# lacibeb/GA3C

Measured on NVIDIA B200. Metric: TPS: A3C training frames/s, NetworkVP 84x84x4 (PPS: predictions/s, in 'pps'), higher is better.
Workload: dtype bf16

## Files before the change

### experiments/microbench/umma_bench.cu

```cuda
#include <cstdio>
#include <cstdlib>
#include <cstdint>
#include <cuda_runtime.h>
#define CK(x) do { cudaError_t e = (x); if (e != cudaSuccess) { printf("CUDA error %s at %d\n", cudaGetErrorString(e), __LINE__); exit(1); } } while (0)

__device__ __forceinline__ uint32_t smem_u32(const void* p) { return (uint32_t)__cvta_generic_to_shared(p); }
__device__ __forceinline__ void mbar_init(uint32_t bar, uint32_t c) { asm volatile("mbarrier.init.shared::cta.b64 [%0], %1;\n" ::"r"(bar), "r"(c)); }
__device__ __forceinline__ void mbar_wait(uint32_t bar, uint32_t parity) {
  asm volatile("{\n.reg .pred p;\nW_%=:\nmbarrier.try_wait.parity.shared::cta.b64 p, [%0], %1;\n@p bra D_%=;\nbra W_%=;\nD_%=:\n}\n" ::"r"(bar), "r"(parity) : "memory");
}
__device__ __forceinline__ bool elect_one() {
  uint32_t pred;
  asm volatile("{\n.reg .pred p;\nelect.sync _|p, 0xffffffff;\nselp.u32 %0, 1, 0, p;\n}\n" : "=r"(pred));
  return pred != 0;
}
__device__ __forceinline__ void mma(uint32_t d, uint32_t a_lo, uint32_t a_hi, uint32_t b_lo, uint32_t b_hi, uint32_t idesc, uint32_t acc) {
  asm volatile("{\n.reg .pred p;\n.reg .b64 da, db;\nsetp.ne.b32 p, %6, 0;\nmov.b64 da, {%1, %2};\nmov.b64 db, {%3, %4};\n"
               "tcgen05.mma.cta_group::1.kind::f16 [%0], da, db, %5, p;\n}\n" ::"r"(d), "r"(a_lo), "r"(a_hi), "r"(b_lo), "r"(b_hi), "r"(idesc), "r"(acc) : "memory");
}
struct Cfg { int M, N, a_mn, b_mn, swz, nacc, a_lbo, a_sbo, b_lbo, b_sbo, a_step, b_step, nrot; };

__global__ void __launch_bounds__(128, 1) bench(Cfg c, int reps, long long* out) {
  extern __shared__ __align__(1024) uint8_t smem[];
  __shared__ __align__(8) unsigned long long bar_s;
  __shared__ uint32_t tslot;
  const uint32_t base = (smem_u32(smem) + 1023u) & ~1023u, bar = smem_u32(&bar_s);
  for (int i = threadIdx.x; i < 200 * 1024 / 16; i += blockDim.x) reinterpret_cast<uint4*>(smem)[i] = make_uint4(0, 0, 0, 0);
  if (threadIdx.x == 0) { mbar_init(bar, 1); asm volatile("fence.mbarrier_init.release.cluster;\n" ::: "memory"); }
  if (threadIdx.x < 32) {
    asm volatile("tcgen05.alloc.cta_group::1.sync.aligned.shared::cta.b32 [%0], 512;\n" ::"r"(smem_u32(&tslot)) : "memory");
    asm volatile("tcgen05.relinquish_alloc_permit.cta_group::1.sync.aligned;\n" ::: "memory");
  }
  asm volatile("fence.proxy.async.shared::cta;\n" ::: "memory");
  asm volatile("tcgen05.fence::before_thread_sync;\n" ::: "memory");
  __syncthreads();
  asm volatile("tcgen05.fence::after_thread_sync;\n" ::: "memory");
  const uint32_t tmem = tslot;
  const uint32_t idesc = (1u << 4) | (1u << 7) | (1u << 10) | ((uint32_t)c.a_mn << 15) | ((uint32_t)c.b_mn << 16) | ((uint32_t)(c.N >> 3) << 17) | ((uint32_t)(c.M >> 4) << 24);
  const uint32_t lay = c.swz ? (2u << 29) : 0u;
  const uint32_t a_base = base, b_base = base + 128 * 1024;
  const uint32_t a_lo0 = ((a_base & 0x3FFFFu) >> 4) | ((uint32_t)(c.a_lbo >> 4) << 16), a_hi = (uint32_t)(c.a_sbo >> 4) | (1u << 14) | lay;
  const uint32_t b_lo0 = ((b_base & 0x3FFFFu) >> 4) | ((uint32_t)(c.b_lbo >> 4) << 16), b_hi = (uint32_t)(c.b_sbo >> 4) | (1u << 14) | lay;
  long long t0 = 0, t1 = 0;
  if (threadIdx.x < 32) {
    for (int round = 0; round < 2; ++round) {
      t0 = clock64();
      if (elect_one()) {
        for (int i = 0; i < reps; ++i) {
          const int r = i % c.nrot;
          mma(tmem + (i % c.nacc) * c.N, a_lo0 + r * (c.a_step >> 4), a_hi, b_lo0 + r * (c.b_step >> 4), b_hi, idesc, 1u);
        }
        asm volatile("tcgen05.commit.cta_group::1.mbarrier::arrive::one.shared::cluster.b64 [%0];\n" ::"r"(bar) : "memory");
      }
      __syncwarp();
      mbar_wait(bar, round & 1);
      t1 = clock64();
    }
  }
  asm volatile("tcgen05.fence::before_thread_sync;\n" ::: "memory");
  __syncthreads();
  if (threadIdx.x == 0) out[blockIdx.x] = t1 - t0;
  if (threadIdx.x < 32) asm volatile("tcgen05.dealloc.cta_group::1.sync.aligned.b32 %0, 512;\n" ::"r"(tmem) : "memory");
}

int main() {
  long long* out; CK(cudaMalloc(&out, 8 * 148));
  CK(cudaFuncSetAttribute(bench, cudaFuncAttributeMaxDynamicSharedMemorySize, 201 * 1024 + 1024));
  const int reps = 2048;
  struct Named { const char* name; Cfg c; } tests[] = {
      {"wgrad11  M64  N16  A MN-ns  B MN-ns  4 acc", {64, 16, 1, 1, 0, 4, 128, 7872, 128, 7424, 256, 256, 16}},
      {"wgrad11  M64  N16  A MN-ns  B MN-ns  1 acc", {64, 16, 1, 1, 0, 1, 128, 7872, 128, 7424, 256, 256, 16}},
      {"wgrad12  M64  N32  A MN-ns  B MN-ns  4 acc", {64, 32, 1, 1, 0, 4, 128, 2560, 128, 2816, 256, 256, 8}},
      {"merged   M64  N64  A MN-ns  B MN-ns  1 acc", {64, 64, 1, 1, 0, 1, 128, 7872, 128, 7424, 256, 256, 16}},
      {"merged   M64  N128 A MN-ns  B MN-ns  1 acc", {64, 128, 1, 1, 0, 1, 128, 7872, 128, 4096, 256, 256, 8}},
      {"         M128 N16  A MN-ns  B MN-ns  4 acc", {128, 16, 1, 1, 0, 4, 128, 7872, 128, 7424, 256, 256, 16}},
      {"         M128 N64  A MN-ns  B MN-ns  1 acc", {128, 64, 1, 1, 0, 1, 128, 7872, 128, 7424, 256, 256, 16}},
      {"dgrad    M128 N64  A K-ns   B K-ns   2 acc", {128, 64, 0, 0, 0, 2, 2816, 128, 1024, 128, 16, 0, 8}},
      {"conv11f  M128 N32  A K-ns   B K-ns   4 acc", {128, 32, 0, 0, 0, 4, 8768, 128, 512, 128, 16, 0, 8}},
      {"         M128 N16  A K-ns   B K-ns   4 acc", {128, 16, 0, 0, 0, 4, 8768, 128, 512, 128, 16, 0, 8}},
      {"         M64  N16  A K-ns   B K-ns   4 acc", {64, 16, 0, 0, 0, 4, 8768, 128, 512, 128, 16, 0, 8}},
      {"conv12f  M128 N32  A K-sw128 B K-sw128 1 acc", {128, 32, 0, 0, 1, 1, 16, 1024, 16, 1024, 32, 32, 4}},
      {"         M128 N64  A K-sw128 B K-sw128 1 acc", {128, 64, 0, 0, 1, 1, 16, 1024, 16, 1024, 32, 32, 4}},
      {"         M128 N128 A K-sw128 B K-sw128 1 acc", {128, 128, 0, 0, 1, 1, 16, 1024, 16, 1024, 32, 32, 4}},
      {"         M128 N256 A K-sw128 B K-sw128 1 acc", {128, 256, 0, 0, 1, 1, 16, 1024, 16, 1024, 32, 32, 4}},
      {"         M64  N32  A K-sw128 B K-sw128 1 acc", {64, 32, 0, 0, 1, 1, 16, 1024, 16, 1024, 32, 32, 4}},
      {"         M64  N64  A MN-sw128 B MN-sw128 1 acc", {64, 64, 1, 1, 1, 1, 8192, 1024, 8192, 1024, 2048, 2048, 4}},
      {"         M64  N16  A MN-sw128 B MN-sw128 4 acc", {64, 16, 1, 1, 1, 4, 8192, 1024, 8192, 1024, 2048, 2048, 4}},
  };
  for (auto& t : tests) {
    bench<<<1, 128, 201 * 1024 + 1024>>>(t.c, reps, out);
    CK(cudaDeviceSynchronize());
    long long cyc; CK(cudaMemcpy(&cyc, out, 8, cudaMemcpyDeviceToHost));
    const double per = (double)cyc / reps;
    const double bytes = (t.c.M * 16 + t.c.N * 16) * 2.0;
    printf("%-52s %7.1f cycles/UMMA   operands %5.0f B -> %5.1f B/clk   %6.1f%% of dense bf16 peak\n", t.name, per, bytes, bytes / per,
           100.0 * (2.0 * t.c.M * t.c.N * 16 / per) / 8192.0);
  }
  return 0;
}
```

### ga3c_b200/csrc/conv_bwd_fused.cu

```cuda
#include "common.cuh"
#include "kernels.h"
#include "tcgen05.cuh"
#include "conv_blk.cuh"
#include "dp_exchange.cuh"

namespace ga3c {

constexpr int FB_THREADS = 512, FB_LOAD_WARP = 0, FB_ISSUE_WARP = 1, FB_C12_WARP = 2, FB_EPI_WARP0 = 4, FB_T1_WARP = 11,
              FB_OPT_WARP0 = 12, FB_OPT_THREADS = FB_THREADS - 32 * FB_OPT_WARP0;
static_assert(FB_EPI_WARP0 % 4 == 0 && FB_T1_WARP % 4 == 3, "an epilogue warp may only read TMEM lane quarter warp % 4");
constexpr int FB_RING = 4;
constexpr int W11_KSTEPS = 31;
constexpr int DN1_ROWS = 16 * W11_KSTEPS, DN1_PLANE = DN1_ROWS * 16, DN1_BYTES = 8 * DN1_PLANE;
constexpr int DG_TILE1 = 28;
constexpr int DG_ROWS = 12 * G_W;
constexpr int W12_KSTEPS = 9;
constexpr int W12D_BYTES = 4 * 4 * 64 * 16;
static_assert(4 * XB_QROWS >= DN1_ROWS && DN1_ROWS >= XB_LIVE_ROWS, "the k-steps must cover every block row");
static_assert(16 * (W12_KSTEPS - 1) + G_W + 1 + 15 < G_ROWS && DG_TILE1 + G_W + 1 + 127 < G_ROWS, "G rows read by the UMMAs");
constexpr int C12_G1 = G_BYTES, C12_B2 = 2 * G_BYTES, C12_BYTES = 2 * G_BYTES + B2_BYTES;

constexpr int FB_OFF_RING = 0;
constexpr int FB_OFF_DN1 = FB_OFF_RING + FB_RING * XB_QBYTES;
constexpr int FB_OFF_C12 = FB_OFF_DN1 + DN1_BYTES;
constexpr int FB_OFF_W12D = FB_OFF_C12 + 2 * C12_BYTES;
constexpr int FB_OFF_RED = FB_OFF_W12D + W12D_BYTES;
constexpr int FB_OFF_BAR = FB_OFF_RED + 5 * C1_OUT * 4;
constexpr int FB_QFULL = 0;
constexpr int FB_QFREE = 4;
constexpr int FB_C12RDY = 8;
constexpr int FB_EPI12 = 10;
constexpr int FB_MMA12 = 12;
constexpr int FB_DN1RDY = 13;
constexpr int FB_DN1FREE = 14;
constexpr int FB_DONE = 15;
constexpr int FB_W12DRDY = 16;
constexpr int FB_NBAR = 17;
constexpr int FB_OFF_TSLOT = FB_OFF_BAR + FB_NBAR * 8;
constexpr int FB_OFF_LAST = FB_OFF_TSLOT + 16;
constexpr int FB_SMEM = FB_OFF_LAST + 16 + 128;
static_assert(FB_SMEM <= 232448, "shared memory budget of one CTA per SM");
constexpr int FB_TMEM_COLS = 512, TM_W11 = 0, TM_W12 = 64, TM_D12 = 192;

template <int DPM, bool EVT>
__global__ void __launch_bounds__(FB_THREADS, 1)
conv_bwd_kernel(const uint8_t* __restrict__ xblk, const uint8_t* __restrict__ n1b2, const uint8_t* __restrict__ dn2g,
                const float* __restrict__ w12, uint16_t* __restrict__ dn1_out, float* __restrict__ g_w11,
                float* __restrict__ g_b11, float* __restrict__ g_w12, float* __restrict__ g_b12, int64_t gp_stride, int batch,
                int n_conv, int hints, const ConvBwdOpt opt, const DpBigArgs dp) {
  constexpr bool DP = DPM != 0;
  if (DPM == 2 && (int)blockIdx.x >= n_conv) {
    griddep_launch();
    griddep_wait(K_DP_BIG);
    dp_big_exchange(dp, (int)blockIdx.x - n_conv, (int)gridDim.x - n_conv);
    trace_mark(K_DP_BIG, 2);
    return;
  }
  extern __shared__ uint8_t smem_raw[];
  const uint32_t sbase = (smem_u32(smem_raw) + 127u) & ~127u;
  uint8_t* const smem = smem_raw + (sbase - smem_u32(smem_raw));
  const uint32_t ring = sbase + FB_OFF_RING, dn1s = sbase + FB_OFF_DN1, c12 = sbase + FB_OFF_C12, w12d = sbase + FB_OFF_W12D,
                 bars = sbase + FB_OFF_BAR, tslot = sbase + FB_OFF_TSLOT;
  float* red = reinterpret_cast<float*>(smem + FB_OFF_RED);
  const int tid = threadIdx.x, warp = tid >> 5, lane = tid & 31;
  EvtLog evt_i = EVT ? evt_open() : EvtLog{nullptr, 0};
  auto mark = [&](int id, int arg) { if (EVT) evt_mark(evt_i, id, arg); };
  const int stride = DPM == 2 ? (int)gridDim.x - dp.n_exch : (int)gridDim.x;
  const int n_frames = ((int)blockIdx.x < batch) ? (batch - 1 - (int)blockIdx.x) / stride + 1 : 0;
  auto frame_of = [&](int k) { return (size_t)(blockIdx.x + k * stride); };
  auto bar = [&](int i) { return bars + i * 8; };
  const uint64_t pol_last_use = (hints & 4) ? l2_policy_evict_first() : l2_policy_normal();

  if (tid == 0) {
    for (int i = 0; i < FB_RING; ++i) { mbar_init(bar(FB_QFULL + i), 1); mbar_init(bar(FB_QFREE + i), 1); }
    for (int p = 0; p < 2; ++p) { mbar_init(bar(FB_C12RDY + p), 1); mbar_init(bar(FB_EPI12 + p), 9); }
    mbar_init(bar(FB_MMA12), 1);
    mbar_init(bar(FB_DN1RDY), 5);
    mbar_init(bar(FB_DN1FREE), 1);
    mbar_init(bar(FB_DONE), 1);
    mbar_init(bar(FB_W12DRDY), 9);
    fence_mbar_init();
  }
  if (warp == FB_EPI_WARP0) tmem_alloc<FB_TMEM_COLS>(tslot);
  for (int i = tid; i < DN1_BYTES / 16; i += FB_THREADS) sts128(dn1s + i * 16, make_uint4(0, 0, 0, 0));
  if (tid < 2) sts128(c12 + tid * C12_BYTES + C12_G1, make_uint4(0, 0, 0, 0));
  fence_proxy_async();
  tc_fence_before();
  __syncthreads();
  tc_fence_after();
  uint32_t tmem_base;
  asm volatile("ld.shared.u32 %0, [%1];\n" : "=r"(tmem_base) : "r"(tslot));
  auto build_w12d = [&]() {
    constexpr int NT = 9 * 32, ITEMS = 4 * 4 * 64, PER = (ITEMS + NT - 1) / NT, UNR = 5;
    static_assert(PER % UNR == 0 || PER < UNR * 4, "unroll chunks");
    const int t = tid - 3 * 32;
#pragma unroll 1
    for (int i0 = 0; i0 < PER; i0 += UNR) {
      float4 lo[UNR], hi[UNR];
#pragma unroll
      for (int u = 0; u < UNR; ++u) {
        const int i = t + (i0 + u) * NT;
        if (i < ITEMS && i0 + u < PER) {
          const int tap = i >> 8, j = (i >> 6) & 3, n = i & 63, a = tap >> 1, b = tap & 1, py = n >> 5, px = (n >> 4) & 1, ci = n & 15;
          const float4* w = reinterpret_cast<const float4*>(w12 + (((py + 2 * a) * 4 + px + 2 * b) * C1_OUT + ci) * C2_OUT + 8 * j);
          lo[u] = w[0]; hi[u] = w[1];
        }
      }
#pragma unroll
      for (int u = 0; u < UNR; ++u) {
        const int i = t + (i0 + u) * NT;
        if (i < ITEMS && i0 + u < PER) {
          const int tap = i >> 8, j = (i >> 6) & 3, n = i & 63;
          sts128(w12d + tap * 4096 + j * 1024 + n * 16,
                 make_uint4(pack_bf16(lo[u].x, lo[u].y), pack_bf16(lo[u].z, lo[u].w), pack_bf16(hi[u].x, hi[u].y), pack_bf16(hi[u].z, hi[u].w)));
        }
      }
    }
    fence_proxy_async();
    __syncwarp();
    if (lane == 0) mbar_arrive(bar(FB_W12DRDY));
    mark(51, 0);
  };
  const bool w12d_early = (hints & 8) != 0;
  if (w12d_early && warp >= 3 && warp <= 11) build_w12d();
  griddep_launch();
  mark(50, 0);
  griddep_wait(K_CONV12_BWD);
  mark(53, 0);
  if (DP && opt.mode != 2 && blockIdx.x == 0 && tid < dp.world) {
    __threadfence_system();
    dp_st_flag(dp.peer[tid] + dp.comm_offset + DPC_BIGREADY + 64 * dp.rank, dp.step);
  }


  auto dgrad_epilogue = [&](int k, int t, int qt, float (&bacc)[C1_OUT]) {
    const uint32_t tlane = tmem_base + ((uint32_t)(qt * 32) << 16);
    const uint32_t b2 = c12 + (k & 1) * C12_BYTES + C12_B2;
    mbar_wait(bar(FB_MMA12), k & 1);
    mark(40, k);
    tc_fence_after();
    uint16_t* dn1_dst = dn1_out ? dn1_out + frame_of(k) * (N1_POS * C1_OUT) : nullptr;
    uint32_t o[4][8];
    int p22[4];
    const int m = (t ? DG_TILE1 : 0) + 32 * qt + lane;
    const int Yh = m / G_W, Xh = m - Yh * G_W;
    const bool row_ok = (t == 0 || m >= 128) && m < DG_ROWS && Xh < 12;
#pragma unroll
    for (int cls = 0; cls < 4; ++cls) {
      uint32_t r[16];
      tc_ld16(tlane + TM_D12 + 64 * t + 16 * cls, r);
      const int y = 2 * Yh + (cls >> 1) - 1, xx = 2 * Xh + (cls & 1) - 1;
      p22[cls] = -1;
      if (row_ok && y >= 0 && y < H1 && xx >= 0 && xx < H1) {
        uint32_t mk[8];
        lds128(*reinterpret_cast<uint32_t(*)[4]>(&mk[0]), b2 + (2 * cls) * B2_LBO + m * 16);
        lds128(*reinterpret_cast<uint32_t(*)[4]>(&mk[4]), b2 + (2 * cls + 1) * B2_LBO + m * 16);
#pragma unroll
        for (int jj = 0; jj < 8; ++jj) {
          const float lo = (mk[jj] & 0x7FFFu) ? __uint_as_float(r[2 * jj]) : 0.f;
          const float hi = (mk[jj] & 0x7FFF0000u) ? __uint_as_float(r[2 * jj + 1]) : 0.f;
          o[cls][jj] = pack_bf16(lo, hi);
          bacc[2 * jj] += bf16_lo(o[cls][jj]);
          bacc[2 * jj + 1] += bf16_hi(o[cls][jj]);
        }
        p22[cls] = y * BLK_W + xx;
        if (dn1_dst) {
          uint4* d = reinterpret_cast<uint4*>(dn1_dst + (y * H1 + xx) * C1_OUT);
          d[0] = make_uint4(o[cls][0], o[cls][1], o[cls][2], o[cls][3]);
          d[1] = make_uint4(o[cls][4], o[cls][5], o[cls][6], o[cls][7]);
        }
      }
    }
    tc_fence_before();
    __syncwarp();
    if (lane == 0) mbar_arrive(bar(FB_EPI12 + (k & 1)));
    mark(43, k);
    if (k > 0) mbar_wait(bar(FB_DN1FREE), (k - 1) & 1);
    mark(41, k);
#pragma unroll
    for (int cls = 0; cls < 4; ++cls) {
      if (p22[cls] >= 0) {
        const uint4 lo4 = make_uint4(o[cls][0], o[cls][1], o[cls][2], o[cls][3]), hi4 = make_uint4(o[cls][4], o[cls][5], o[cls][6], o[cls][7]);
        const uint32_t dst = dn1s + p22[cls] * 16;
#pragma unroll
        for (int ab = 0; ab < 4; ++ab) {
          const uint32_t d = dst + (2 * ab) * DN1_PLANE + (BLK_W * (ab >> 1) + (ab & 1)) * 16;
          sts128(d, lo4);
          sts128(d + DN1_PLANE, hi4);
        }
      }
    }
    fence_proxy_async();
    __syncwarp();
    if (lane == 0) mbar_arrive(bar(FB_DN1RDY));
    mark(42, k);
  };
  auto b11_partial = [&](int slot, const float (&bacc)[C1_OUT]) {
#pragma unroll
    for (int c = 0; c < C1_OUT; ++c) {
      float v = bacc[c];
#pragma unroll
      for (int o = 16; o > 0; o >>= 1) v += __shfl_xor_sync(0xffffffffu, v, o);
      if (lane == 0) red[slot * C1_OUT + c] = v;
    }
  };

  if (warp == FB_LOAD_WARP) {
    const int n_q = n_frames * XB_QUARTERS;
    for (int qg = 0; qg < n_q; ++qg) {
      const int slot = qg % FB_RING, use = qg / FB_RING;
      mark(1, qg);
      if (use > 0) mbar_wait(bar(FB_QFREE + slot), (use - 1) & 1);
      mark(2, qg);
      if (elect_one()) {
        const int k = qg >> 2, q = qg & 3;
        mbar_expect_tx(bar(FB_QFULL + slot), XB_QBYTES);
        bulk_load_hint(ring + slot * XB_QBYTES, xblk + frame_of(k) * XB_FRAME_BYTES + q * XB_QBYTES, XB_QBYTES, bar(FB_QFULL + slot),
                       pol_last_use);
      }
      __syncwarp();
    }
  } else if (warp == FB_C12_WARP) {
    for (int k = 0; k < n_frames; ++k) {
      const int p = k & 1;
      mark(20, k);
      if (k >= 2) mbar_wait(bar(FB_EPI12 + p), ((k >> 1) - 1) & 1);
      mark(21, k);
      if (elect_one()) {
        const uint32_t buf = c12 + p * C12_BYTES;
        mbar_expect_tx(bar(FB_C12RDY + p), 2 * G_BYTES - 16 + B2_BYTES);
        bulk_load(buf, dn2g + frame_of(k) * G_BYTES, G_BYTES, bar(FB_C12RDY + p));
        bulk_load_hint(buf + C12_G1 + 16, dn2g + frame_of(k) * G_BYTES, G_BYTES - 16, bar(FB_C12RDY + p), pol_last_use);
        bulk_load_hint(buf + C12_B2, n1b2 + frame_of(k) * B2_BYTES, B2_BYTES, bar(FB_C12RDY + p), pol_last_use);
      }
      __syncwarp();
    }
  } else if (warp == FB_ISSUE_WARP) {
    constexpr uint32_t idesc_dg = make_idesc_m(128, 64, false, false), idesc_w12 = make_idesc_m(64, 2 * C2_OUT, true, true),
                       idesc_w11 = make_idesc_m(64, 4 * C1_OUT, true, true);
    const uint32_t wd_k = desc_ns_lo(w12d, 1024);
    const uint32_t ring_mn = desc_ns_lo(ring, 128), dn1_mn = desc_ns_lo(dn1s, 128);
    constexpr uint32_t hi_k = desc_ns_hi(128), hi_g = desc_ns_hi(G_LBO), hi_b2 = desc_ns_hi(B2_LBO), hi_ring = desc_ns_hi(XB_PLANE_BYTES),
                       hi_dn1 = desc_ns_hi(DN1_PLANE);
    mbar_wait(bar(FB_W12DRDY), 0);
    auto conv12_mmas = [&](int k) {
      const int p = k & 1;
      const uint32_t buf = c12 + p * C12_BYTES;
      const uint32_t g_k = desc_ns_lo(buf, G_LBO), g_mn = desc_ns_lo(buf, 128), b2_mn = desc_ns_lo(buf + C12_B2, 128);
      mark(10, k);
      mbar_wait(bar(FB_C12RDY + p), (k >> 1) & 1);
      if (k > 0) mbar_wait(bar(FB_EPI12 + (p ^ 1)), ((k - 1) >> 1) & 1);
      mark(11, k);
      tc_fence_after();
      if (elect_one()) {
#pragma unroll
        for (int t = 0; t < 2; ++t)
#pragma unroll
          for (int tap = 0; tap < 4; ++tap)
#pragma unroll
            for (int kk = 0; kk < 2; ++kk)
              tc_mma_bf16_w(tmem_base + TM_D12 + 64 * t,
                            g_k + ((t ? DG_TILE1 : 0) + G_W + 1 - G_W * (tap >> 1) - (tap & 1)) + 2 * kk * (G_LBO / 16), hi_k,
                            wd_k + (tap * 4096 + 2 * kk * 1024) / 16, hi_k, idesc_dg, (tap | kk) ? 1u : 0u);
        const uint32_t acc = k ? 1u : 0u;
#pragma unroll
        for (int s = 0; s < W12_KSTEPS; ++s)
#pragma unroll
          for (int a = 0; a < 2; ++a)
            tc_mma_bf16_w(tmem_base + TM_W12 + 64 * a, b2_mn + 16 * s, hi_b2, g_mn + 16 * s + G_W + 1 - G_W * a, hi_g,
                          idesc_w12, s ? 1u : acc);
        tc_commit(bar(FB_MMA12));
      }
      __syncwarp();
      mark(12, k);
    };
    auto conv11_mmas = [&](int k) {
      mark(13, k);
      mbar_wait(bar(FB_DN1RDY), k & 1);
      mark(14, k);
#pragma unroll 1
      for (int q = 0; q < XB_QUARTERS; ++q) {
        const int qg = k * XB_QUARTERS + q, slot = qg % FB_RING;
        mbar_wait(bar(FB_QFULL + slot), (qg / FB_RING) & 1);
        mark(15, qg);
        tc_fence_after();
        if (elect_one()) {
          const int n_kk = q == 3 ? W11_KSTEPS - 24 : 8;
          for (int kk = 0; kk < n_kk; ++kk) {
            const int s = 8 * q + kk;
            tc_mma_bf16_w(tmem_base + TM_W11, ring_mn + slot * (XB_QBYTES / 16) + kk * 16, hi_ring, dn1_mn + 16 * s, hi_dn1,
                          idesc_w11, (k | s) ? 1u : 0u);
          }
          tc_commit(bar(FB_QFREE + slot));
          if (q == 3) tc_commit(bar(FB_DN1FREE));
        }
        __syncwarp();
        mark(16, qg);
      }
    };
    if (n_frames > 0) conv12_mmas(0);
    if (n_frames > 1) conv12_mmas(1);
    for (int k = 0; k < n_frames; ++k) {
      conv11_mmas(k);
      if (k + 2 < n_frames) conv12_mmas(k + 2);
    }
    if (elect_one()) tc_commit(bar(FB_DONE));
    __syncwarp();
  } else if (warp >= FB_OPT_WARP0) {
    const int t = tid - 32 * FB_OPT_WARP0;
    if (opt.mode == 1) {
      const long long stride4 = (long long)n_conv * FB_OPT_THREADS;
      const float one_m_rho = 1.f - opt.decay;
      const bool has_mom = opt.momentum != 0.f;
      const float4* g4 = reinterpret_cast<const float4*>(opt.g);
      float4* w4 = reinterpret_cast<float4*>(opt.w);
      float4* ms4 = reinterpret_cast<float4*>(opt.ms);
      float4* mom4 = reinterpret_cast<float4*>(opt.mom);
      uint2* sh = reinterpret_cast<uint2*>(opt.shadow);
      constexpr int U = 4;
#pragma unroll 1
      for (long long i0 = (long long)blockIdx.x * FB_OPT_THREADS + t; i0 < opt.n4; i0 += U * stride4) {
        float4 gv[U], wv[U], mv[U];
#pragma unroll
        for (int u = 0; u < U; ++u) {
          const long long i = i0 + u * stride4;
          if (i < opt.n4) { gv[u] = __ldcg(g4 + i); wv[u] = w4[i]; mv[u] = ms4[i]; }
        }
#pragma unroll
        for (int u = 0; u < U; ++u) {
          const long long i = i0 + u * stride4;
          if (i >= opt.n4) continue;
          float4 mo = has_mom ? mom4[i] : make_float4(0.f, 0.f, 0.f, 0.f);
#define GA3C_RMS(c)                                                          \
  mv[u].c = opt.decay * mv[u].c + one_m_rho * gv[u].c * gv[u].c;             \
  mo.c = opt.momentum * mo.c + opt.lr * gv[u].c / sqrtf(mv[u].c + opt.eps);  \
  wv[u].c -= mo.c;
          GA3C_RMS(x) GA3C_RMS(y) GA3C_RMS(z) GA3C_RMS(w)
#undef GA3C_RMS
          w4[i] = wv[u];
          ms4[i] = mv[u];
          if (has_mom) mom4[i] = mo;
          sh[i] = make_uint2(pack_bf16(wv[u].x, wv[u].y), pack_bf16(wv[u].z, wv[u].w));
        }
      }
    } else if (DPM == 2 && opt.mode == 2) {
      dp_big_group(dp, t, FB_OPT_THREADS, (int)blockIdx.x, n_conv, 4, reinterpret_cast<int*>(smem + FB_OFF_LAST), true);
    }
  } else if (warp == FB_T1_WARP) {
    if (!w12d_early) build_w12d();
    float bacc11[C1_OUT];
#pragma unroll
    for (int c = 0; c < C1_OUT; ++c) bacc11[c] = 0.f;
    for (int k = 0; k < n_frames; ++k) dgrad_epilogue(k, 1, 3, bacc11);
    b11_partial(4, bacc11);
  } else if (warp == 3 || warp >= 8) {
    if (!w12d_early) build_w12d();
    const int j = warp == 3 ? 3 : warp - 8;
    float acc8[8];
#pragma unroll
    for (int e = 0; e < 8; ++e) acc8[e] = 0.f;
    for (int k = 0; k < n_frames; ++k) {
      const int p = k & 1;
      mbar_wait(bar(FB_C12RDY + p), (k >> 1) & 1);
      mark(30, k);
      const uint32_t plane = c12 + p * C12_BYTES + j * G_LBO;
      for (int row = lane; row < G_ROWS; row += 32) {
        uint32_t v[4];
        lds128(v, plane + row * 16);
#pragma unroll
        for (int e = 0; e < 4; ++e) { acc8[2 * e] += bf16_lo(v[e]); acc8[2 * e + 1] += bf16_hi(v[e]); }
      }
      __syncwarp();
      if (lane == 0) mbar_arrive(bar(FB_EPI12 + p));
    }
#pragma unroll
    for (int e = 0; e < 8; ++e) {
      float v = acc8[e];
#pragma unroll
      for (int o = 16; o > 0; o >>= 1) v += __shfl_xor_sync(0xffffffffu, v, o);
      if (lane == 0) g_b12[(int64_t)blockIdx.x * gp_stride + 8 * j + e] = v;
    }
  } else {
    if (!w12d_early) build_w12d();
    const int ew = warp - FB_EPI_WARP0;
    const uint32_t tlane = tmem_base + ((uint32_t)(ew * 32) << 16);
    float bacc[C1_OUT];
#pragma unroll
    for (int c = 0; c < C1_OUT; ++c) bacc[c] = 0.f;
    for (int k = 0; k < n_frames; ++k) dgrad_epilogue(k, 0, ew, bacc);
    b11_partial(ew, bacc);
    if (n_frames > 0) {
      mbar_wait(bar(FB_DONE), 0);
      mark(54, 0);
      tc_fence_after();
      float* const s11 = g_w11 + (int64_t)blockIdx.x * gp_stride;
      float* const s12 = g_w12 + (int64_t)blockIdx.x * gp_stride;
      const int row = 16 * ew + lane, j = row >> 3, e = row & 7;
#pragma unroll 1
      for (int q = 0; q < 4; ++q) {
        uint32_t r[16];
        tc_ld16(tlane + TM_W11 + 16 * q, r);
        if (lane < 16) {
          const int kh = 4 * (q >> 1) + (j >> 1), kw = 4 * (q & 1) + (j & 1) * 2 + (e >> 2), c = e & 3;
          float4* o = reinterpret_cast<float4*>(s11 + ((kh * 8 + kw) * 4 + c) * C1_OUT);
#pragma unroll
          for (int n = 0; n < C1_OUT / 4; ++n)
            o[n] = make_float4(__uint_as_float(r[4 * n]), __uint_as_float(r[4 * n + 1]), __uint_as_float(r[4 * n + 2]),
                               __uint_as_float(r[4 * n + 3]));
        }
      }
#pragma unroll 1
      for (int q = 0; q < 4; ++q)
#pragma unroll 1
        for (int hh = 0; hh < 2; ++hh) {
          uint32_t r[16];
          tc_ld16(tlane + TM_W12 + 64 * (q >> 1) + 32 * (q & 1) + 16 * hh, r);
          if (lane < 16) {
            const int kh = 2 * (q >> 1) + (j >> 2), kw = 2 * (q & 1) + ((j >> 1) & 1), ci = (j & 1) * 8 + e;
            float4* o = reinterpret_cast<float4*>(s12 + ((kh * 4 + kw) * C1_OUT + ci) * C2_OUT + 16 * hh);
#pragma unroll
            for (int n = 0; n < 4; ++n)
              o[n] = make_float4(__uint_as_float(r[4 * n]), __uint_as_float(r[4 * n + 1]), __uint_as_float(r[4 * n + 2]),
                                 __uint_as_float(r[4 * n + 3]));
          }
        }
    }
  }

  mark(52, 0);
  tc_fence_before();
  __syncthreads();
  if (tid < C1_OUT)
    g_b11[(int64_t)blockIdx.x * gp_stride + tid] =
        red[tid] + red[C1_OUT + tid] + red[2 * C1_OUT + tid] + red[3 * C1_OUT + tid] + red[4 * C1_OUT + tid];
  trace_mark(K_CONV12_BWD, 2);
  if (warp == FB_EPI_WARP0) {
    tc_fence_after();
    tmem_dealloc<FB_TMEM_COLS>(tmem_base);
  }
}

GA3C_TRACE_ATTACH(trace_attach_conv_bwd_fused)
static bool g_evt_attached = false;
int evt_attach_conv_bwd(unsigned long long* buf) {
  g_evt_attached = buf != nullptr;
  return (int)cudaMemcpyToSymbol(g_evt, &buf, sizeof(buf));
}

int conv_bwd_grid(int batch, int num_sms, int n_exch) { return min(batch, num_sms - n_exch); }

int configure_conv_bwd_fused() {
  cudaError_t e = cudaFuncSetAttribute(conv_bwd_kernel<0, false>, cudaFuncAttributeMaxDynamicSharedMemorySize, FB_SMEM);
  if (e != cudaSuccess) return (int)e;
  e = cudaFuncSetAttribute(conv_bwd_kernel<0, true>, cudaFuncAttributeMaxDynamicSharedMemorySize, FB_SMEM);
  if (e != cudaSuccess) return (int)e;
  e = cudaFuncSetAttribute(conv_bwd_kernel<1, false>, cudaFuncAttributeMaxDynamicSharedMemorySize, FB_SMEM);
  if (e != cudaSuccess) return (int)e;
  return (int)cudaFuncSetAttribute(conv_bwd_kernel<2, false>, cudaFuncAttributeMaxDynamicSharedMemorySize, FB_SMEM);
}

int launch_conv_bwd(const uint8_t* xblk, const uint8_t* n1b2, const uint8_t* dn2g, const float* w12, uint16_t* dn1_out,
                    float* g_w11, float* g_b11, float* g_w12, float* g_b12, int64_t gp_stride, int batch, int num_sms, bool x_u8,
                    const ConvBwdOpt& opt, const DpBigArgs* dp, cudaStream_t stream) {
  DpBigArgs d{};
  if (dp != nullptr) d = *dp;
  const int n_conv = conv_bwd_grid(batch, num_sms, d.n_exch);
  const dim3 grid(n_conv + d.n_exch);
  if (grid.x == 0) return 0;
  if (opt.mode == 2 && (dp == nullptr || n_conv == 0)) return (int)cudaErrorInvalidValue;
  auto kernel = dp != nullptr ? ((d.n_exch > 0 || opt.mode == 2) ? conv_bwd_kernel<2, false> : conv_bwd_kernel<1, false>)
                              : (g_evt_attached ? conv_bwd_kernel<0, true> : conv_bwd_kernel<0, false>);
  return launch_pdl(kernel, grid, dim3(FB_THREADS), FB_SMEM, stream, xblk, n1b2, dn2g, w12, dn1_out, g_w11, g_b11, g_w12, g_b12,
                    gp_stride, batch, n_conv, l2_hints(true, x_u8) | (batch >= num_sms ? 8 : 0), opt, d);
}

}
```

Measured before the change: 10.43 million.

## Transpose conv dgrad UMMA to M64xN144 and spread epilogue over eight warps

The dgrad UMMA is recomputed as a transposed product: one M64 x N144 tile with weights as A and G as B, replacing two M128 x N64 tiles that overlapped. This cuts redundant MMA work. The epilogue is redistributed across eight warps, each handling one pixel class and five 16-column groups, using shuffle transposes. The four bias-12 reduction warps are merged into warp 3, and the dn1 planes get a 16-byte bank skew. The tradeoff is extra shuffle work in the epilogue and new lane-to-channel mapping logic, which adds a risk of indexing errors.

```diff
diff --git a/experiments/microbench/umma_bench.cu b/experiments/microbench/umma_bench.cu
--- a/experiments/microbench/umma_bench.cu
+++ b/experiments/microbench/umma_bench.cu
@@ -86,6 +86,9 @@
       {"         M64  N32  A K-sw128 B K-sw128 1 acc", {64, 32, 0, 0, 1, 1, 16, 1024, 16, 1024, 32, 32, 4}},
       {"         M64  N64  A MN-sw128 B MN-sw128 1 acc", {64, 64, 1, 1, 1, 1, 8192, 1024, 8192, 1024, 2048, 2048, 4}},
       {"         M64  N16  A MN-sw128 B MN-sw128 4 acc", {64, 16, 1, 1, 1, 4, 8192, 1024, 8192, 1024, 2048, 2048, 4}},
+      {"dgradT   M64  N144 A K-ns   B K-ns   1 acc", {64, 144, 0, 0, 0, 1, 1024, 128, 2752, 128, 0, 16, 8}},
+      {"dgradT   M64  N160 A K-ns   B K-ns   1 acc", {64, 160, 0, 0, 0, 1, 1024, 128, 2752, 128, 0, 16, 8}},
+      {"wgrad12  M64  N128 A MN-ns  B MN-ns  1 acc", {64, 128, 1, 1, 0, 1, 128, 2560, 128, 2752, 256, 256, 8}},
   };
   for (auto& t : tests) {
     bench<<<1, 128, 201 * 1024 + 1024>>>(t.c, reps, out);
diff --git a/ga3c_b200/csrc/conv_bwd_fused.cu b/ga3c_b200/csrc/conv_bwd_fused.cu
--- a/ga3c_b200/csrc/conv_bwd_fused.cu
+++ b/ga3c_b200/csrc/conv_bwd_fused.cu
@@ -6,18 +6,22 @@
 
 namespace ga3c {
 
-constexpr int FB_THREADS = 512, FB_LOAD_WARP = 0, FB_ISSUE_WARP = 1, FB_C12_WARP = 2, FB_EPI_WARP0 = 4, FB_T1_WARP = 11,
-              FB_OPT_WARP0 = 12, FB_OPT_THREADS = FB_THREADS - 32 * FB_OPT_WARP0;
-static_assert(FB_EPI_WARP0 % 4 == 0 && FB_T1_WARP % 4 == 3, "an epilogue warp may only read TMEM lane quarter warp % 4");
+constexpr int FB_THREADS = 512, FB_LOAD_WARP = 0, FB_ISSUE_WARP = 1, FB_C12_WARP = 2, FB_EPI_WARP0 = 4, FB_OPT_WARP0 = 12,
+              FB_OPT_THREADS = FB_THREADS - 32 * FB_OPT_WARP0;
+static_assert(FB_EPI_WARP0 % 4 == 0, "an epilogue warp may only read TMEM lane quarter warp % 4");
 constexpr int FB_RING = 4;
 constexpr int W11_KSTEPS = 31;
-constexpr int DN1_ROWS = 16 * W11_KSTEPS, DN1_PLANE = DN1_ROWS * 16, DN1_BYTES = 8 * DN1_PLANE;
-constexpr int DG_TILE1 = 28;
-constexpr int DG_ROWS = 12 * G_W;
+constexpr int DN1_ROWS = 16 * W11_KSTEPS, DN1_PLANE = DN1_ROWS * 16 + 16, DN1_BYTES = 8 * DN1_PLANE;
+static_assert(DN1_PLANE % 128 == 16, "bank skew of the dn1 planes");
+constexpr int DG_N = 144;
+__host__ __device__ constexpr int dg_lane_ci(int l) { return (l & 3) | ((l & 4) << 1) | ((l & 8) >> 1); }
+constexpr int DG_GPW = 5;
+static_assert(2 * 16 * DG_GPW >= DG_N, "the two epilogue warps of a class cover D^T");
 constexpr int W12_KSTEPS = 9;
 constexpr int W12D_BYTES = 4 * 4 * 64 * 16;
 static_assert(4 * XB_QROWS >= DN1_ROWS && DN1_ROWS >= XB_LIVE_ROWS, "the k-steps must cover every block row");
-static_assert(16 * (W12_KSTEPS - 1) + G_W + 1 + 15 < G_ROWS && DG_TILE1 + G_W + 1 + 127 < G_ROWS, "G rows read by the UMMAs");
+static_assert(DG_N % 16 == 0 && DG_N <= 256 && (H1 / 2) * G_W + H1 / 2 < DG_N, "D^T must cover every position with a live pixel");
+static_assert(16 * (W12_KSTEPS - 1) + G_W + 1 + 15 < G_ROWS && G_W + 1 + DG_N - 1 < G_ROWS, "G rows read by the UMMAs");
 constexpr int C12_G1 = G_BYTES, C12_B2 = 2 * G_BYTES, C12_BYTES = 2 * G_BYTES + B2_BYTES;
 
 constexpr int FB_OFF_RING = 0;
@@ -25,7 +29,7 @@
 constexpr int FB_OFF_C12 = FB_OFF_DN1 + DN1_BYTES;
 constexpr int FB_OFF_W12D = FB_OFF_C12 + 2 * C12_BYTES;
 constexpr int FB_OFF_RED = FB_OFF_W12D + W12D_BYTES;
-constexpr int FB_OFF_BAR = FB_OFF_RED + 5 * C1_OUT * 4;
+constexpr int FB_OFF_BAR = FB_OFF_RED + 8 * C1_OUT * 4;
 constexpr int FB_QFULL = 0;
 constexpr int FB_QFREE = 4;
 constexpr int FB_C12RDY = 8;
@@ -41,6 +45,7 @@
 constexpr int FB_SMEM = FB_OFF_LAST + 16 + 128;
 static_assert(FB_SMEM <= 232448, "shared memory budget of one CTA per SM");
 constexpr int FB_TMEM_COLS = 512, TM_W11 = 0, TM_W12 = 64, TM_D12 = 192;
+static_assert(TM_D12 + DG_N <= FB_TMEM_COLS, "TMEM columns");
 
 template <int DPM, bool EVT>
 __global__ void __launch_bounds__(FB_THREADS, 1)
@@ -75,7 +80,7 @@
     for (int i = 0; i < FB_RING; ++i) { mbar_init(bar(FB_QFULL + i), 1); mbar_init(bar(FB_QFREE + i), 1); }
     for (int p = 0; p < 2; ++p) { mbar_init(bar(FB_C12RDY + p), 1); mbar_init(bar(FB_EPI12 + p), 9); }
     mbar_init(bar(FB_MMA12), 1);
-    mbar_init(bar(FB_DN1RDY), 5);
+    mbar_init(bar(FB_DN1RDY), 8);
     mbar_init(bar(FB_DN1FREE), 1);
     mbar_init(bar(FB_DONE), 1);
     mbar_init(bar(FB_W12DRDY), 9);
@@ -101,7 +106,8 @@
       for (int u = 0; u < UNR; ++u) {
         const int i = t + (i0 + u) * NT;
         if (i < ITEMS && i0 + u < PER) {
-          const int tap = i >> 8, j = (i >> 6) & 3, n = i & 63, a = tap >> 1, b = tap & 1, py = n >> 5, px = (n >> 4) & 1, ci = n & 15;
+          const int tap = i >> 8, j = (i >> 6) & 3, n = i & 63, a = tap >> 1, b = tap & 1, py = n >> 5, px = (n >> 4) & 1,
+                    ci = dg_lane_ci(n & 15);
           const float4* w = reinterpret_cast<const float4*>(w12 + (((py + 2 * a) * 4 + px + 2 * b) * C1_OUT + ci) * C2_OUT + 8 * j);
           lo[u] = w[0]; hi[u] = w[1];
         }
@@ -133,42 +139,59 @@
   }
 
 
-  auto dgrad_epilogue = [&](int k, int t, int qt, float (&bacc)[C1_OUT]) {
-    const uint32_t tlane = tmem_base + ((uint32_t)(qt * 32) << 16);
+  auto dgrad_epilogue = [&](int k, int cls, int g0, float (&bacc)[8]) {
+    const uint32_t tlane = tmem_base + ((uint32_t)(cls * 32) << 16);
     const uint32_t b2 = c12 + (k & 1) * C12_BYTES + C12_B2;
     mbar_wait(bar(FB_MMA12), k & 1);
     mark(40, k);
     tc_fence_after();
     uint16_t* dn1_dst = dn1_out ? dn1_out + frame_of(k) * (N1_POS * C1_OUT) : nullptr;
-    uint32_t o[4][8];
-    int p22[4];
-    const int m = (t ? DG_TILE1 : 0) + 32 * qt + lane;
-    const int Yh = m / G_W, Xh = m - Yh * G_W;
-    const bool row_ok = (t == 0 || m >= 128) && m < DG_ROWS && Xh < 12;
-#pragma unroll
-    for (int cls = 0; cls < 4; ++cls) {
+    const int h = (lane >> 2) & 1, e8 = ((lane >> 1) & 4) | (lane & 3);
+    auto pixel_row = [&](int gi) {
+      const int m = 16 * gi + (lane & 16 ? 8 : 0) + e8;
+      const int Yh = m / G_W, Xh = m - Yh * G_W;
+      const int y = 2 * Yh + (cls >> 1) - 1, xx = 2 * Xh + (cls & 1) - 1;
+      return Xh < 12 && y >= 0 && y < H1 && xx >= 0 && xx < H1 ? y * BLK_W + xx : -1;
+    };
+    uint32_t o[DG_GPW][4];
+#pragma unroll
+    for (int li = 0; li < DG_GPW; ++li) {
+      const int gi = g0 + li;
+      if (gi >= DG_N / 16) break;
       uint32_t r[16];
-      tc_ld16(tlane + TM_D12 + 64 * t + 16 * cls, r);
-      const int y = 2 * Yh + (cls >> 1) - 1, xx = 2 * Xh + (cls & 1) - 1;
-      p22[cls] = -1;
-      if (row_ok && y >= 0 && y < H1 && xx >= 0 && xx < H1) {
-        uint32_t mk[8];
-        lds128(*reinterpret_cast<uint32_t(*)[4]>(&mk[0]), b2 + (2 * cls) * B2_LBO + m * 16);
-        lds128(*reinterpret_cast<uint32_t(*)[4]>(&mk[4]), b2 + (2 * cls + 1) * B2_LBO + m * 16);
-#pragma unroll
-        for (int jj = 0; jj < 8; ++jj) {
-          const float lo = (mk[jj] & 0x7FFFu) ? __uint_as_float(r[2 * jj]) : 0.f;
-          const float hi = (mk[jj] & 0x7FFF0000u) ? __uint_as_float(r[2 * jj + 1]) : 0.f;
-          o[cls][jj] = pack_bf16(lo, hi);
-          bacc[2 * jj] += bf16_lo(o[cls][jj]);
-          bacc[2 * jj + 1] += bf16_hi(o[cls][jj]);
-        }
-        p22[cls] = y * BLK_W + xx;
-        if (dn1_dst) {
-          uint4* d = reinterpret_cast<uint4*>(dn1_dst + (y * H1 + xx) * C1_OUT);
-          d[0] = make_uint4(o[cls][0], o[cls][1], o[cls][2], o[cls][3]);
-          d[1] = make_uint4(o[cls][4], o[cls][5], o[cls][6], o[cls][7]);
-        }
+      tc_ld16(tlane + TM_D12 + 16 * gi, r);
+      float v[8];
+#pragma unroll
+      for (int j = 0; j < 8; ++j) {
+        const uint32_t up = __shfl_sync(0xffffffffu, r[8 + j], lane & 15);
+        v[j] = __uint_as_float(lane < 16 ? r[j] : up);
+      }
+#pragma unroll
+      for (int d = 4; d > 0; d >>= 1) {
+        const int ld = d == 4 ? 8 : d;
+        const bool hi_side = (lane & ld) != 0;
+#pragma unroll
+        for (int j = 0; j < 8; ++j) {
+          if (j & d) continue;
+          const float x = __shfl_xor_sync(0xffffffffu, hi_side ? v[j] : v[j | d], ld);
+          if (hi_side) v[j] = x; else v[j | d] = x;
+        }
+      }
+      const int p22 = pixel_row(gi);
+      if (p22 >= 0) {
+        const int m = 16 * gi + (lane & 16 ? 8 : 0) + e8, y = p22 / BLK_W, xx = p22 - y * BLK_W;
+        uint32_t mk[4];
+        lds128(mk, b2 + (2 * cls + h) * B2_LBO + m * 16);
+#pragma unroll
+        for (int jj = 0; jj < 4; ++jj) {
+          const float lo = (mk[jj] & 0x7FFFu) ? v[2 * jj] : 0.f;
+          const float hi = (mk[jj] & 0x7FFF0000u) ? v[2 * jj + 1] : 0.f;
+          o[li][jj] = pack_bf16(lo, hi);
+          bacc[2 * jj] += bf16_lo(o[li][jj]);
+          bacc[2 * jj + 1] += bf16_hi(o[li][jj]);
+        }
+        if (dn1_dst)
+          *reinterpret_cast<uint4*>(dn1_dst + (y * H1 + xx) * C1_OUT + 8 * h) = make_uint4(o[li][0], o[li][1], o[li][2], o[li][3]);
       }
     }
     tc_fence_before();
@@ -178,16 +201,16 @@
     if (k > 0) mbar_wait(bar(FB_DN1FREE), (k - 1) & 1);
     mark(41, k);
 #pragma unroll
-    for (int cls = 0; cls < 4; ++cls) {
-      if (p22[cls] >= 0) {
-        const uint4 lo4 = make_uint4(o[cls][0], o[cls][1], o[cls][2], o[cls][3]), hi4 = make_uint4(o[cls][4], o[cls][5], o[cls][6], o[cls][7]);
-        const uint32_t dst = dn1s + p22[cls] * 16;
-#pragma unroll
-        for (int ab = 0; ab < 4; ++ab) {
-          const uint32_t d = dst + (2 * ab) * DN1_PLANE + (BLK_W * (ab >> 1) + (ab & 1)) * 16;
-          sts128(d, lo4);
-          sts128(d + DN1_PLANE, hi4);
-        }
+    for (int li = 0; li < DG_GPW; ++li) {
+      const int gi = g0 + li;
+      if (gi >= DG_N / 16) break;
+      const int p22 = pixel_row(gi);
+      if (p22 >= 0) {
+        const uint4 c4 = make_uint4(o[li][0], o[li][1], o[li][2], o[li][3]);
+        const uint32_t dst = dn1s + h * DN1_PLANE + p22 * 16;
+#pragma unroll
+        for (int ab = 0; ab < 4; ++ab)
+          sts128(dst + (2 * ab) * DN1_PLANE + (BLK_W * (ab >> 1) + (ab & 1)) * 16, c4);
       }
     }
     fence_proxy_async();
@@ -195,13 +218,15 @@
     if (lane == 0) mbar_arrive(bar(FB_DN1RDY));
     mark(42, k);
   };
-  auto b11_partial = [&](int slot, const float (&bacc)[C1_OUT]) {
-#pragma unroll
-    for (int c = 0; c < C1_OUT; ++c) {
+  auto b11_partial = [&](int slot, const float (&bacc)[8]) {
+#pragma unroll
+    for (int c = 0; c < 8; ++c) {
       float v = bacc[c];
-#pragma unroll
-      for (int o = 16; o > 0; o >>= 1) v += __shfl_xor_sync(0xffffffffu, v, o);
-      if (lane == 0) red[slot * C1_OUT + c] = v;
+      v += __shfl_xor_sync(0xffffffffu, v, 16);
+      v += __shfl_xor_sync(0xffffffffu, v, 8);
+      v += __shfl_xor_sync(0xffffffffu, v, 2);
+      v += __shfl_xor_sync(0xffffffffu, v, 1);
+      if ((lane & 27) == 0) red[slot * C1_OUT + 8 * (lane >> 2) + c] = v;
     }
   };
 
@@ -236,7 +261,7 @@
       __syncwarp();
     }
   } else if (warp == FB_ISSUE_WARP) {
-    constexpr uint32_t idesc_dg = make_idesc_m(128, 64, false, false), idesc_w12 = make_idesc_m(64, 2 * C2_OUT, true, true),
+    constexpr uint32_t idesc_dg = make_idesc_m(64, DG_N, false, false), idesc_w12 = make_idesc_m(64, 2 * C2_OUT, true, true),
                        idesc_w11 = make_idesc_m(64, 4 * C1_OUT, true, true);
     const uint32_t wd_k = desc_ns_lo(w12d, 1024);
     const uint32_t ring_mn = desc_ns_lo(ring, 128), dn1_mn = desc_ns_lo(dn1s, 128);
@@ -254,14 +279,11 @@
       tc_fence_after();
       if (elect_one()) {
 #pragma unroll
-        for (int t = 0; t < 2; ++t)
-#pragma unroll
-          for (int tap = 0; tap < 4; ++tap)
-#pragma unroll
-            for (int kk = 0; kk < 2; ++kk)
-              tc_mma_bf16_w(tmem_base + TM_D12 + 64 * t,
-                            g_k + ((t ? DG_TILE1 : 0) + G_W + 1 - G_W * (tap >> 1) - (tap & 1)) + 2 * kk * (G_LBO / 16), hi_k,
-                            wd_k + (tap * 4096 + 2 * kk * 1024) / 16, hi_k, idesc_dg, (tap | kk) ? 1u : 0u);
+        for (int tap = 0; tap < 4; ++tap)
+#pragma unroll
+          for (int kk = 0; kk < 2; ++kk)
+            tc_mma_bf16_w(tmem_base + TM_D12, wd_k + (tap * 4096 + 2 * kk * 1024) / 16, hi_k,
+                          g_k + (G_W + 1 - G_W * (tap >> 1) - (tap & 1)) + 2 * kk * (G_LBO / 16), hi_k, idesc_dg, (tap | kk) ? 1u : 0u);
         const uint32_t acc = k ? 1u : 0u;
 #pragma unroll
         for (int s = 0; s < W12_KSTEPS; ++s)
@@ -346,50 +368,53 @@
     } else if (DPM == 2 && opt.mode == 2) {
       dp_big_group(dp, t, FB_OPT_THREADS, (int)blockIdx.x, n_conv, 4, reinterpret_cast<int*>(smem + FB_OFF_LAST), true);
     }
-  } else if (warp == FB_T1_WARP) {
+  } else if (warp == 3) {
     if (!w12d_early) build_w12d();
-    float bacc11[C1_OUT];
-#pragma unroll
-    for (int c = 0; c < C1_OUT; ++c) bacc11[c] = 0.f;
-    for (int k = 0; k < n_frames; ++k) dgrad_epilogue(k, 1, 3, bacc11);
-    b11_partial(4, bacc11);
-  } else if (warp == 3 || warp >= 8) {
-    if (!w12d_early) build_w12d();
-    const int j = warp == 3 ? 3 : warp - 8;
-    float acc8[8];
-#pragma unroll
-    for (int e = 0; e < 8; ++e) acc8[e] = 0.f;
+    float acc8[4][8];
+#pragma unroll
+    for (int j = 0; j < 4; ++j)
+#pragma unroll
+      for (int e = 0; e < 8; ++e) acc8[j][e] = 0.f;
     for (int k = 0; k < n_frames; ++k) {
       const int p = k & 1;
       mbar_wait(bar(FB_C12RDY + p), (k >> 1) & 1);
       mark(30, k);
-      const uint32_t plane = c12 + p * C12_BYTES + j * G_LBO;
-      for (int row = lane; row < G_ROWS; row += 32) {
-        uint32_t v[4];
-        lds128(v, plane + row * 16);
-#pragma unroll
-        for (int e = 0; e < 4; ++e) { acc8[2 * e] += bf16_lo(v[e]); acc8[2 * e + 1] += bf16_hi(v[e]); }
+#pragma unroll
+      for (int j = 0; j < 4; ++j) {
+        const uint32_t plane = c12 + p * C12_BYTES + j * G_LBO;
+#pragma unroll
+        for (int i = 0; i < (G_ROWS + 31) / 32; ++i) {
+          const int row = lane + 32 * i;
+          if (row < G_ROWS) {
+            uint32_t v[4];
+            lds128(v, plane + row * 16);
+#pragma unroll
+            for (int e = 0; e < 4; ++e) { acc8[j][2 * e] += bf16_lo(v[e]); acc8[j][2 * e + 1] += bf16_hi(v[e]); }
+          }
+        }
       }
       __syncwarp();
       if (lane == 0) mbar_arrive(bar(FB_EPI12 + p));
     }
 #pragma unroll
-    for (int e = 0; e < 8; ++e) {
-      float v = acc8[e];
-#pragma unroll
-      for (int o = 16; o > 0; o >>= 1) v += __shfl_xor_sync(0xffffffffu, v, o);
-      if (lane == 0) g_b12[(int64_t)blockIdx.x * gp_stride + 8 * j + e] = v;
-    }
+    for (int j = 0; j < 4; ++j)
+#pragma unroll
+      for (int e = 0; e < 8; ++e) {
+        float v = acc8[j][e];
+#pragma unroll
+        for (int o = 16; o > 0; o >>= 1) v += __shfl_xor_sync(0xffffffffu, v, o);
+        if (lane == 0) g_b12[(int64_t)blockIdx.x * gp_stride + 8 * j + e] = v;
+      }
   } else {
     if (!w12d_early) build_w12d();
-    const int ew = warp - FB_EPI_WARP0;
+    const int ew = warp & 3;
     const uint32_t tlane = tmem_base + ((uint32_t)(ew * 32) << 16);
-    float bacc[C1_OUT];
-#pragma unroll
-    for (int c = 0; c < C1_OUT; ++c) bacc[c] = 0.f;
-    for (int k = 0; k < n_frames; ++k) dgrad_epilogue(k, 0, ew, bacc);
-    b11_partial(ew, bacc);
-    if (n_frames > 0) {
+    float bacc[8];
+#pragma unroll
+    for (int c = 0; c < 8; ++c) bacc[c] = 0.f;
+    for (int k = 0; k < n_frames; ++k) dgrad_epilogue(k, ew, warp >= 8 ? DG_GPW : 0, bacc);
+    b11_partial(warp - FB_EPI_WARP0, bacc);
+    if (warp < 8 && n_frames > 0) {
       mbar_wait(bar(FB_DONE), 0);
       mark(54, 0);
       tc_fence_after();
@@ -430,9 +455,12 @@
   mark(52, 0);
   tc_fence_before();
   __syncthreads();
-  if (tid < C1_OUT)
-    g_b11[(int64_t)blockIdx.x * gp_stride + tid] =
-        red[tid] + red[C1_OUT + tid] + red[2 * C1_OUT + tid] + red[3 * C1_OUT + tid] + red[4 * C1_OUT + tid];
+  if (tid < C1_OUT) {
+    float s = red[tid];
+#pragma unroll
+    for (int w = 1; w < 8; ++w) s += red[w * C1_OUT + tid];
+    g_b11[(int64_t)blockIdx.x * gp_stride + tid] = s;
+  }
   trace_mark(K_CONV12_BWD, 2);
   if (warp == FB_EPI_WARP0) {
     tc_fence_after();
```

Result: no change. 10.35 million (median of 6 runs) (-0.8%).
